# mlelarge/graph_neural_net

Hardware: AMD Instinct MI355X
Metric: graph-pairs/sec FGNN fwd+bwd, N=50 regular pairs (higher is better)
Workload: dtype f32

## Files before the change

### graph_neural_net_amd/_lib.py

```python
import ctypes as C
import os

import torch

_HERE = os.path.dirname(os.path.abspath(__file__))
LIB_PATH = os.environ.get('FGNN_LIB') or os.path.join(_HERE, 'libfgnn_hip.so')

FGNN_H = 32
FGNN_TILE = 32
FGNN_MAX_DEPTH = 3
FGNN_RANGE_WG = 256
FGNN_LSAP_MAX_N = 2048
FGNN_MAX_LEVELS = 64
FGNN_QAP_MAX_N = 256
FGNN_QAPW_MAX_N = 256
FGNN_SEED_MAX_N = 256
FGNN_SINKHORN_LDS_MAX_N = 192
FGNN_RESTART_STREAM = 9
FGNN_RESTART_MAX_R = 64
FGNN_RESTART_MAX_STARTS = 65535
FGNN_SPECTRAL_MAX_N = 256
FGNN_SPECTRAL_MAX_POWERS = 8
FGNN_PLANTED_MAX_N = 256
FGNN_SCORE_SPLIT = 4
# ... 54 lines not shown

class MlpBwdArgs(C.Structure):
    _fields_ = [('G', C.c_int), ('N', C.c_int), ('depth', C.c_int),
                ('nvalid', C.c_void_p),
                ('a', Slab), ('b', Slab),
                ('W', C.c_void_p * FGNN_MAX_DEPTH),
                ('bias', C.c_void_p * FGNN_MAX_DEPTH),
                ('dy', C.c_void_p), ('dgstride', C.c_longlong), ('ldd', C.c_longlong),
                ('z', C.c_void_p), ('zgstride', C.c_longlong), ('ldz', C.c_longlong),
                ('coef', C.c_void_p), ('s12', C.c_void_p), ('znrm', C.c_void_p),
                ('dxa', C.c_void_p), ('dxa_gstride', C.c_longlong), ('dxa_ld', C.c_longlong),
                ('dxb', C.c_void_p), ('dxb_gstride', C.c_longlong), ('dxb_ld', C.c_longlong),
                ('accumulate_a', C.c_int), ('accumulate_b', C.c_int),
                ('wpart', C.c_void_p), ('s12part', C.c_void_p), ('packed', C.c_void_p),
                ('s12tiles', C.c_void_p), ('s12_out', C.c_void_p), ('xbits', C.c_void_p), ('xdeg', C.c_void_p),
                ('ranges', C.c_void_p), ('cu_share', C.c_int)]


class Slab16(C.Structure):
    _fields_ = [('ptr', C.c_void_p), ('gstride', C.c_longlong), ('ldp', C.c_longlong), ('C', C.c_int),
                ('nrm', C.c_void_p), ('beta', C.c_void_p)]


class MlpFwd16Args(C.Structure):
    _fields_ = [('G', C.c_int), ('N', C.c_int), ('ldr', C.c_int), ('depth', C.c_int), ('nmlp', C.c_int),
                ('nvalid', C.c_void_p),
                ('a', Slab16), ('b', Slab16),
                ('z', C.c_void_p * 2), ('ldz', C.c_longlong),
                ('part', C.c_void_p * 2), ('cnt', C.c_void_p), ('packed', C.c_void_p), ('ranges', C.c_void_p)]


# ... 151 lines not shown
    'fgnn_block1_struct_supported': [_I, _I, _I],
    'fgnn_block1_struct_table_floats': [_I],
    'fgnn_block1_struct_ws_floats': [_I, _I],
    'fgnn_block1_struct_rows': [_I, _I],
    'fgnn_block1_struct_fwd': [_VP, _VP, _I, _I, _VP, _VP, _VP, _VP, _VP, C.c_float, _VP, _VP, _VP, _LL, _LL, _VP, _VP, _VP, _VP, _VP, _VP, _VP],
    'fgnn_block1_struct_bwd': [_VP, _VP, _I, _I, _VP, _VP, _VP, _VP, _VP, _VP, _VP, _VP, _LL, _LL, _VP, _VP, _VP, _VP, _VP, _VP],
    'fgnn_block1_struct_fwd_pack': [_VP, _VP, _I, _I, _VP, _VP, _VP, _VP, _VP, C.c_float, _VP, _VP, _VP, _LL, _LL, _VP, _VP, _VP, _VP, _VP, _VP, _VP, _I, _VP],
    'fgnn_block1_struct_fwd16_pack': [_VP, _VP, _I, _I, _I, _VP, _VP, _VP, _VP, _VP, C.c_float, _VP, _VP, _VP, _LL, _LL, _VP, _VP, _VP, _VP, _VP, _VP, _VP, _I, _VP],
    'fgnn_block1_struct_fwd16': [_VP, _VP, _I, _I, _I, _VP, _VP, _VP, _VP, _VP, C.c_float, _VP, _VP, _VP, _LL, _LL, _VP, _VP, _VP, _VP, _VP, _VP, _VP],
    'fgnn_block1_struct_bwd16': [_VP, _VP, _I, _I, _I, _VP, _VP, _VP, _VP, _VP, _VP, _VP, _VP, _LL, _LL, _VP, _VP, _VP, _VP, _VP, _VP],
    'fgnn_mlp_bwd_coef_tiles_supported': [_I, _I],
    'fgnn_mlp_param_count': [_I, _I],
    'fgnn_reduce_partials': [_VP, _I, _I, _VP, _VP],
    'fgnn_chan_matmul_bwd': [C.POINTER(Slab), C.POINTER(Slab), _VP, _LL, _LL, _VP, _I, _I, _VP, _VP, _LL, _LL, _VP, _VP, _VP],
    'fgnn_chan_matmul_bwd_ord': [C.POINTER(Slab), C.POINTER(Slab), _VP, _LL, _LL, _VP, _I, _I, _VP, _VP, _LL, _LL, _VP, _VP, _VP, _I, _VP],
    'fgnn_sum_scale': [_VP, _I, _I, _F, _VP, _VP],
    'fgnn_adam_step': [_VP, _VP, _VP, _VP, _I, C.c_double, C.c_double, C.c_double, C.c_double, _I, C.c_double, _VP],
    'fgnn_adam_step_dev': [_VP, _VP, _VP, _VP, _I, _VP, _VP, _VP],
    'fgnn_grad_guard': [_VP, _I, _VP, _VP, _VP],
    'fgnn_adam_step_guarded': [_VP, _VP, _VP, _VP, _I, _VP, _VP, _VP, _VP],
    'fgnn_expand_adjacency': [_VP, _VP, _I, _I, _VP, _VP],
    'fgnn_pack_adjacency': [_VP, _VP, _I, _I, _VP, _VP, _VP],
    'fgnn_pack_adjacency_ld': [_VP, _VP, _I, _I, _I, _VP, _VP, _VP],
    'fgnn_pack_adjacency_pair': [_VP, _VP, _VP, _VP, _I, _I, _I, _VP, _VP, _VP, _VP, _VP],
    'fgnn_adjacency_degree': [_VP, _VP, _I, _I, _VP, _VP],
    'fgnn_accuracy_max': [_VP, _VP, _I, _I, _VP, _VP],
    'fgnn_lsap_accuracy': [_VP, _LL, _I, _VP, _I, _I, _VP, _VP, _VP],
    'fgnn_pairgen_supported': [_I, _I, _I],
    'fgnn_pairgen': [C.POINTER(PairgenArgs), _VP],
    'fgnn_pairgen_indexed': [C.POINTER(PairgenArgs), _VP, _VP],
# ... 170 lines not shown
```

### graph_neural_net_amd/csrc/fgnn_bwd32.h

```cpp
#pragma once
#include "fgnn_common.h"

namespace {

constexpr int BWD_WG = 256;
constexpr int NW = 8;
constexpr int NP = 4;
static_assert(BWD_WG == FGNN_RANGE_WG, "fgnn_ragged_tile_ranges splits for the backward grid");

DEVI float4 coef_from_sums(const float4 n, const float2 sv, float nv) {
    const float m = nv * nv;
    float4 k;
    k.x = n.x;
    k.y = n.y;
    k.z = m > 0.f ? -n.y * sv.y * n.w / m : 0.f;
    k.w = m > 0.f ? -n.y * sv.x / m : 0.f;
    return k;
}
DEVI float4 coef_record(const fgnn_mlp_bwd_args &A, int g, int ch, int nv) {
    if (A.coef) return reinterpret_cast<const float4 *>(A.coef)[(long long)g * FGNN_H + ch];
    const float4 n = reinterpret_cast<const float4 *>(A.znrm)[(long long)g * FGNN_H + ch];
    const float2 sv = reinterpret_cast<const float2 *>(A.s12)[(long long)g * FGNN_H + ch];
    return coef_from_sums(n, sv, (float)nv);
}
// ... 35 lines not shown
        const int m = e >= PCOUNT / 4 ? 1 : 0, ee = e - m * (PCOUNT / 4);
        float4 a = part4[(4 * m) * (PCOUNT / 4) + ee];
#pragma unroll
        for (int w = 1; w < NP; ++w) {
            const float4 b = part4[(4 * m + w) * (PCOUNT / 4) + ee];
            a.x += b.x;
            a.y += b.y;
            a.z += b.z;
            a.w += b.w;
        }
        reinterpret_cast<float4 *>(P.m[m].wpart + (long long)blockIdx.x * PCOUNT)[ee] = a;
    }
}

inline int check_mlp_bwd_common(const fgnn_mlp_bwd_args *a, const char *fn, int tile_bits) {
    FGNN_CHECK(a->dy && a->z && a->wpart, "%s: missing dy/z/wpart", fn);
    FGNN_CHECK(a->coef || (a->s12 && a->znrm) || (a->s12tiles && a->znrm), "%s: need coef, or s12 + znrm, or s12tiles + znrm", fn);
    const long long lim = 0x7fffffffll / 4, G = a->G;
    FGNN_CHECK(G * a->a.gstride < lim && G * a->b.gstride < lim && G * a->dgstride < lim && G * a->zgstride < lim &&
               G * a->dxa_gstride < lim && G * a->dxb_gstride < lim,
               "%s: a tensor exceeds 2 GiB (32-bit buffer addressing); split the batch", fn);
    FGNN_CHECK(G * fgnn_tiles_per_graph(a->N) < (1ll << tile_bits), "%s: too many tiles", fn);
    FGNN_CHECK(BWD_WG == fgnn_mlp_bwd_num_workgroups(), "%s: workgroup count differs from fgnn_mlp_bwd", fn);
    return 0;
}
inline int check_pair_common(const fgnn_mlp_bwd_args *a1, const fgnn_mlp_bwd_args *a2, const char *fn, int tile_bits, bool dense_only) {
    FGNN_CHECK(a1 && a2, "%s: null args", fn);
    FGNN_CHECK(BWD_WG == fgnn_mlp_bwd_num_workgroups(), "%s: workgroup count differs from fgnn_mlp_bwd", fn);
    FGNN_CHECK(a1->G > 0 && a1->N > 0 && a1->G == a2->G && a1->N == a2->N && a1->depth == a2->depth,
               "%s: the two MLPs must share G, N and depth", fn);
    FGNN_CHECK((!dense_only || a1->a.ptr) && a1->a.ptr == a2->a.ptr && a1->a.C == a2->a.C && a1->a.gstride == a2->a.gstride &&
               a1->a.ldp == a2->a.ldp && a1->a.nrm == a2->a.nrm && a1->a.beta == a2->a.beta &&
               (dense_only || (a1->xbits == a2->xbits && a1->xdeg == a2->xdeg)) && a1->nvalid == a2->nvalid,
               "%s: the two MLPs must read the same input slab", fn);
    FGNN_CHECK(!a1->dxa && !a1->s12part, "%s: the input gradient and its tile sums belong to the SECOND argument block", fn);
    FGNN_CHECK(!a1->s12tiles && !a2->s12tiles, "%s: s12tiles is an mlp3 feature", fn);
    for (const fgnn_mlp_bwd_args *a : {a1, a2}) {
        FGNN_CHECK(a->dy && a->z && a->wpart, "%s: missing dy/z/wpart", fn);
        FGNN_CHECK(a->coef || (a->s12 && a->znrm), "%s: need coef, or s12 + znrm", fn);
        const long long lim = 0x7fffffffll / 4, G = a->G;
        FGNN_CHECK(G * a->a.gstride < lim && G * a->dgstride < lim && G * a->zgstride < lim && G * a->dxa_gstride < lim,
                   "%s: a tensor exceeds 2 GiB (32-bit buffer addressing); split the batch", fn);
    }
    FGNN_CHECK((long long)a1->G * fgnn_tiles_per_graph(a1->N) < (1ll << tile_bits), "%s: too many tiles", fn);
    return 0;
}

}
```

### graph_neural_net_amd/csrc/fgnn_bwd_t16.h

```cpp
#pragma once
#include "fgnn_t16.h"
#include "fgnn_pack.h"
#include "fgnn_bwd32.h"

namespace {

using namespace t16;

template <int CB, int IMAGES, int NSLOTS>
struct BwdT16Layout {
    static constexpr int DEPTH = 3;
    static constexpr PkBwd PK = pk_bwd(32, CB, DEPTH);
    static constexpr int OFF_W1 = PK.off_wh, OFF_WT1 = PK.off_wt, OFF_WT2 = PK.off_wt + 16;
    static constexpr int BIAS_F = PK.bias_f;
    static constexpr int WEIGHT_F = pk_pad_floats(PK.floats);
    static constexpr int NSLOT = NSLOTS;
    static constexpr int CIN = 32 + CB;
    static constexpr int PCOUNT = 32 * CIN + 32 + (DEPTH - 1) * (32 * 32 + 32);
    static constexpr int TILE_OFF = IMAGES * WEIGHT_F;
    static constexpr int TILE_END = TILE_OFF + NW * NSLOT * TILE_F;
    static constexpr int RED_F = NW * PCOUNT;
};


#define FGNN_T16_READ_RECORDS(norm)                                 \
    _Pragma("unroll") for (int s = 0; s < 8; ++s) {                 \
        const float4 k4 = rec[chan_s(s) + chan_q(q)];               \
        kx[s] = k4.x;                                               \
        ky[s] = k4.y;                                               \
        kz[s] = k4.z;                                               \
        kw[s] = k4.w;                                               \
        if (norm) {                                                 \
            const float4 n = rec[32 + chan_s(s) + chan_q(q)];       \
            mean[s] = n.x;                                          \
            av[s] = n.y;                                            \
        }                                                           \
    }

#define FGNN_T16_RECOMPUTE_HIDDEN(acc, h1, h2)                                              \
    _Pragma("unroll") for (int s = 0; s < 8; ++s) h1[s] = relu1(acc[s >> 2][s & 3]);        \
    stage8(S0, lane_base, h1);                                                              \
    load_bias(acc, wl + L::BIAS_F, 1, q);                                                   \
    gemm32<L::OFF_W1>(acc, wl, h1, lane);                                                   \
    _Pragma("unroll") for (int s = 0; s < 8; ++s) h2[s] = relu1(acc[s >> 2][s & 3]);        \
    stage8(S1, lane_base, h2);

#define FGNN_T16_DZ(dpre)                                                                                                   \
    _Pragma("unroll") for (int s = 0; s < 8; ++s) dpre[s] = fmaf(kz[s], zr[s] - kx[s], fmaf(ky[s], dyr[s], kw[s]));         \
    if (!full) {                                                                                                            \
        _Pragma("unroll") for (int s = 0; s < 8; ++s) dpre[s] = valid ? dpre[s] : 0.f;                                      \
    }

#define FGNN_T16_HIDDEN_BWD(OFF_WT, dpre, dW, db, Dt, In, h)                                                \
    {                                                                                                       \
        f32x4 a2[2];                                                                                        \
        a2[0] = a2[1] = zero4();                                                                            \
        gemm32<OFF_WT>(a2, wl, dpre, lane);                                                                 \
        wgrad16(dW, db, Dt, In, lane);                                                                      \
        _Pragma("unroll") for (int s = 0; s < 8; ++s) dpre[s] = h[s] > 0.f ? a2[s >> 2][s & 3] : 0.f;       \
    }

#define FGNN_T16_DB_BUTTERFLY(db0, db1, db2)            \
    _Pragma("unroll") for (int b = 0; b < 2; ++b) {     \
// ... 10 lines not shown
```

### graph_neural_net_amd/csrc/matmul.hip

```cpp
#include "fgnn_common.h"
#include "fgnn_norm.h"

namespace {

constexpr int TM = 64;
constexpr int LDS_LD = 65;

DEVI void stage_tile(float *lds, const float *mat, int N, int nv, int row0, int col0, const NormRec &nr, int tid) {
    if (row0 == 0 && col0 == 0 && N <= TM) {
        for (int e = tid; e < TM * TM; e += 256) lds[(e >> 6) * LDS_LD + (e & 63)] = 0.f;
        __syncthreads();
        const int P = N * N;
        for (int e = tid; e < P; e += 256) {
            const int r = e / N, c = e - r * N;
            float v = mat[e];
            const bool ok = r < nv && c < nv;
            v = ok ? (nr.on ? (v - nr.mean) * nr.a + nr.beta : v) : 0.f;
            lds[r * LDS_LD + c] = v;
        }
    } else {
        for (int e = tid; e < TM * TM; e += 256) {
            const int r = e >> 6, c = e & 63;
            const int gr = row0 + r, gc = col0 + c;
            float v = 0.f;
// ... 188 lines not shown
template <bool WANT_S>
DEVI void tile_to_global(const View &ov, int mat_off4, const float *lds, int N, const float (&u)[16], float &s1,
                         float &s2, int tid) {
    const int c = tid & 63, r0 = __builtin_amdgcn_readfirstlane(tid >> 6);
    const int voff = c < N ? (r0 * N + c) * 4 : OOB_OFF;
    const float *lp = lds + r0 * LDS_LD + c;
#pragma unroll
    for (int k = 0; k < 16; ++k) {
        const float t = lp[4 * k * LDS_LD];
        buf_store(t, ov, r0 + 4 * k < N ? voff : OOB_OFF, mat_off4 + k * 16 * N);
        if (WANT_S) {
            s1 += t;
            s2 += t * u[k];
        }
    }
}

DEVI void load_tile_raw(float (&x)[16], const View &v, int mat_off4, int N, int nv, int tid) {
    const int c = tid & 63, r0 = __builtin_amdgcn_readfirstlane(tid >> 6);
    const int voff = c < nv ? (r0 * N + c) * 4 : OOB_OFF;
#pragma unroll
    for (int k = 0; k < 16; ++k) {
        const int r = r0 + 4 * k;
        x[k] = buf_load(v, r < nv ? voff : OOB_OFF, mat_off4 + k * 16 * N);
    }
}
template <bool WANT_U>
DEVI void finish_tile(float (&v)[16], float (&u)[16], const float (&x)[16], int nv, const NormRec &nr, int tid) {
#pragma unroll
    for (int k = 0; k < 16; ++k) {
// ... 65 lines not shown
#pragma unroll
        for (int r = 0; r < 16; ++r) acc[r] = 0.f;
        if (32 * qi < N && 32 * qj < N) {
            const float *ap = As + (32 * qi + j) * LDS_LD + h;
            const float *bp = Bs + h * LDS_LD + 32 * qj + j;
            for (int k = 0; k < N; k += 2) acc = mfma32(ap[k], bp[k * LDS_LD], acc);
        }
        __syncthreads();
        frag_to_lds(As, 32 * qi, 32 * qj, acc, lane);
        __syncthreads();
        float s1 = 0.f, s2 = 0.f;
        tile_to_global<false>(vO, o_off, As, N, dummy, s1, s2, tid);
    }
}

__global__ __launch_bounds__(256, 4) void chan_matmul_bwd1_kernel(const fgnn_slab ya, const fgnn_slab yb,
                                                               const float *dm, long long dmg, long long ldm,
                                                               const int *nvalid, int N, int M, float *da, float *db,
                                                               long long ogstride, long long ldo, float *s12a,
                                                               float *s12b) {
    __shared__ float Bs[TM * LDS_LD];
    __shared__ float Ds[TM * LDS_LD];
    __shared__ float red[4][4];
    const int C = ya.C;
    const int tid = threadIdx.x, lane = tid & 63, wave = tid >> 6;
    const int qi = wave >> 1, qj = wave & 1;
    const int j = lane & 31, h = lane >> 5;
    NormRec none;
    none.on = false; none.mean = 0.f; none.a = 1.f; none.beta = 0.f;
    float xa[16], xb[16], xd[16], dummy[16];
// ... 33 lines not shown
            for (int k = 0; k < N; k += 2) accA = mfma32(ap[k], bp[k], accA);
        }
        __syncthreads();
        store_tile_lds(Bs, va, tid);
        __syncthreads();
        if (live) {
            const float *ap = Bs + h * LDS_LD + 32 * qi + j;
            const float *bp = Ds + h * LDS_LD + 32 * qj + j;
            for (int k = 0; k < N; k += 2) accB = mfma32(ap[k * LDS_LD], bp[k * LDS_LD], accB);
        }
        __syncthreads();
        frag_to_lds(Ds, 32 * qi, 32 * qj, accA, lane);
        frag_to_lds(Bs, 32 * qi, 32 * qj, accB, lane);
        __syncthreads();
        float sa1 = 0.f, sa2 = 0.f, sb1 = 0.f, sb2 = 0.f;
        if (s12a) {
            tile_to_global<true>(vOA, o_off, Ds, N, ua, sa1, sa2, tid);
            tile_to_global<true>(vOB, o_off, Bs, N, ub, sb1, sb2, tid);
            s12_epilogue(red, sa1, sa2, sb1, sb2, s12a, s12b, gc, tid);
        } else {
            tile_to_global<false>(vOA, o_off, Ds, N, dummy, sa1, sa2, tid);
            tile_to_global<false>(vOB, o_off, Bs, N, dummy, sb1, sb2, tid);
        }
    }
}


int g_mm_wave_variant = 1;
inline bool mm_wave_variant() { return (g_mm_wave_variant & 1) != 0; }
inline bool mm_narrow() { return (g_mm_wave_variant & 8) != 0; }
constexpr int WLD = 68;
// ... 654 lines not shown
extern "C" int fgnn_chan_matmul_bwd_ord(const fgnn_slab *ya, const fgnn_slab *yb, const float *dm, long long dmgstride,
                                        long long ldm, const int *nvalid, int G, int N, float *da, float *db,
                                        long long ogstride, long long ldo, float *s12a, float *s12b, const int *order,
                                        int fill, void *stream) {
    FGNN_CHECK(!order || nvalid, "fgnn_chan_matmul_bwd_ord: an order needs the nvalid it was derived from");
    FGNN_CHECK(ya && yb && dm && da && db && ya->ptr && yb->ptr, "fgnn_chan_matmul_bwd: null argument");
    FGNN_CHECK(ya->C == yb->C && ya->C > 0 && G > 0 && N > 0, "fgnn_chan_matmul_bwd: bad shapes");
    FGNN_CHECK((s12a == nullptr) == (s12b == nullptr), "fgnn_chan_matmul_bwd: s12a and s12b come together");
    FGNN_CHECK(!s12a || (ya->nrm && yb->nrm), "fgnn_chan_matmul_bwd: s12 outputs need normalised slabs");
    const int t = (N + TM - 1) / TM;
    const bool fused = s12a && t == 1;
    if (t == 1) {
        if (check_2gib("fgnn_chan_matmul_bwd", G, ya->gstride, yb->gstride, dmgstride)) return 1;
        FGNN_CHECK((long long)G * ogstride < 0x7fffffffll / 4, "fgnn_chan_matmul_bwd: output exceeds 2 GiB");
        const int M = G * ya->C;
        hipLaunchKernelGGL(chan_matmul_bwd1_kernel, dim3(M), dim3(256), 0, (hipStream_t)stream, *ya, *yb, dm,
                           dmgstride, ldm, nvalid, N, M, da, db, ogstride, ldo, s12a, s12b);
        FGNN_LAUNCH_CHECK();
        return 0;
    }
    if (big_path(N)) {
        if (check_2gib("fgnn_chan_matmul_bwd", G, ya->gstride, yb->gstride, dmgstride, ogstride)) return 1;
#define FGNN_BIG_BWD(MT)                                                                                              \
    {                                                                                                                 \
        static LdsAttrCache attr_cache;                                                                           \
        (void)fgnn_raise_lds(attr_cache, (const void *)chan_matmul_bwd_big_kernel<MT>, BigCfg<MT>::LDS_BYTES);                   \
        hipLaunchKernelGGL(chan_matmul_bwd_big_kernel<MT>, dim3(G * ya->C * (split ? 2 : 1)), dim3(BIG_THREADS),      \
                           BigCfg<MT>::LDS_BYTES, (hipStream_t)stream, *ya, *yb, dm, dmgstride, ldm, nvalid, N, G, da, \
                           db, ogstride, ldo, s12a, s12b, order, split, fill);                                            \
    }
        const int split = (order && (long long)G * ya->C <= BIG_SPLIT_MAX_MATRICES) ? 1 : 0;
// ... 2 lines not shown
#undef FGNN_BIG_BWD
        FGNN_LAUNCH_CHECK();
        return 0;
    }
    hipLaunchKernelGGL(chan_matmul_bwd_kernel, dim3(t, t, G * ya->C), dim3(256), 0, (hipStream_t)stream, *ya, *yb, dm,
                       dmgstride, ldm, nvalid, N, da, db, ogstride, ldo, fused ? s12a : nullptr, fused ? s12b : nullptr);
    FGNN_LAUNCH_CHECK();
    if (s12a && !fused) {
        int rc = fgnn_gn_bwd_stats(da, ogstride, ldo, ya->ptr, ya->gstride, ya->ldp, ya->nrm, nvalid, G, ya->C, N, s12a, stream);
        if (rc) return rc;
        rc = fgnn_gn_bwd_stats(db, ogstride, ldo, yb->ptr, yb->gstride, yb->ldp, yb->nrm, nvalid, G, yb->C, N, s12b, stream);
        if (rc) return rc;
    }
    return 0;
}
```

### graph_neural_net_amd/csrc/mlp_bwd_pair_t16.hip

```cpp
#include "fgnn_bwd_t16.h"

#ifdef FGNN_PHASES
__device__ unsigned long long *g_phase16_buf = nullptr;
#define PH_DECL unsigned long long ph_[16] = {0, 0, 0, 0, 0, 0, 0, 0, 0, 0, 0, 0, 0, 0, 0, 0}; unsigned long long ph_last_ = __builtin_amdgcn_s_memtime();
#define PH(k) { const unsigned long long t_ = __builtin_amdgcn_s_memtime(); ph_[k] += t_ - ph_last_; ph_last_ = t_; }
#define PH_FLUSH if (g_phase16_buf && (threadIdx.x & 63) == 0) { for (int k_ = 0; k_ < 16; ++k_) g_phase16_buf[((long long)blockIdx.x * NW + wv) * 16 + k_] = ph_[k_]; }
#else
#define PH_DECL
#define PH(k)
#define PH_FLUSH
#endif

namespace {

struct PairLayout16 : BwdT16Layout<0, 2, 4> {
    static constexpr int OFF_W0 = PK.off_w1a, OFF_WT0 = PK.off_wt0a;
    static constexpr int XCH_OFF = TILE_END;
    static constexpr int FLAG_OFF = XCH_OFF + NP * 1024;
    static constexpr int REC_OFF = FLAG_OFF + 4 * NP;
    static constexpr int LIVE_OFF = REC_OFF + NW * 256;
    static constexpr int MAIN_F = LIVE_OFF + LIVE_LIST_CAP + NW;
    static constexpr int LDS_F = MAIN_F > RED_F ? MAIN_F : RED_F;
};

template <bool SKIP, bool HAS_DX>
__global__ __launch_bounds__(64 * NW, 2) void mlp_bwd_pair_t16_kernel(const PairArgs P, const int tpg, const int total_tiles) {
    extern __shared__ __attribute__((aligned(16))) float smem[];
    using L = PairLayout16;
    const int lane = threadIdx.x & 63, wv = __builtin_amdgcn_readfirstlane(threadIdx.x >> 6);
    const int role = wv >> 2, pair = wv & 3;
    const int px = lane & 15, q = lane >> 4;
    const fgnn_mlp_bwd_args &A = P.m[role];
    const int P2 = A.N * A.N;
    const View va = make_view(A.a.ptr, A.a.gstride, A.a.ldp, A.G);
    const View vdy = make_view(A.dy, A.dgstride, A.ldd, A.G);
    const View vz = make_view(A.z, A.zgstride, A.ldz, A.G);
    const View vdx = make_view(P.m[1].dxa, P.m[1].dxa_gstride, P.m[1].dxa_ld, P.m[1].G);

    PH_DECL
    if (role == 1) __builtin_amdgcn_s_setprio(1);
// ... 23 lines not shown
    pk_glds<NW>(smem, P.m[0].packed, L::WEIGHT_F, wv, lane);
    pk_glds<NW>(smem + L::WEIGHT_F, P.m[1].packed, L::WEIGHT_F, wv, lane);
    PH(15)

    float mean[8], av[8], beta[8], kx[8], ky[8], kz[8], kw[8];
#pragma unroll
    for (int s = 0; s < 8; ++s) {
        mean[s] = 0.f;
        av[s] = 1.f;
        beta[s] = normA && A.a.beta ? A.a.beta[chan(s, 0) + chan_q(q)] : 0.f;
        kx[s] = ky[s] = kz[s] = kw[s] = 0.f;
    }
    float4 *rec = reinterpret_cast<float4 *>(smem + L::REC_OFF) + wv * 64;
    auto fetch_records = [&](int g, int nv) {
        if (lane < 32) {
            rec[lane] = coef_record(A, g, lane, nv);
            if (normA) rec[32 + lane] = reinterpret_cast<const float4 *>(A.a.nrm)[(long long)g * A.a.C + lane];
        }
    };
    auto read_records = [&]() { FGNN_T16_READ_RECORDS(normA) };

    float xa[8], dyr[8], zr[8], oldr[8];
#pragma unroll
    for (int s = 0; s < 8; ++s) oldr[s] = 0.f;
    int cached_g = -1, cur_nv = A.N;
    int tile = T0 + pair;
    int live_cnt = 0;
    if constexpr (SKIP) tile = __builtin_amdgcn_readfirstlane(next_owned_live_tile_p(T0, T1, live_cnt, pair, NP, tpg, FGNN_TILE, A.N, A.nvalid));
    int hf = 0;
    {
        const bool act = tile < T1;
        const int g = __builtin_amdgcn_readfirstlane(act ? tile / tpg : 0);
        const int p = (act ? tile - g * tpg : 0) * 32 + px;
        const bool inb0 = act && p < P2;
        load8(xa, va, lane_voff(va, q, p, inb0), g * va.gs4);
// ... 5 lines not shown
    }
    PH(12)
    if (threadIdx.x < 4 * NP) reinterpret_cast<int *>(smem + L::FLAG_OFF)[threadIdx.x] = 0;
    PH(13)
    int *live_list = reinterpret_cast<int *>(smem + L::LIVE_OFF);
    int nlive = 0, li = pair;
    if constexpr (SKIP) nlive = build_live_list(live_list, live_list + LIVE_LIST_CAP, T0, T1, tpg, FGNN_TILE, A.N, A.nvalid, threadIdx.x, 64 * NW);
    const bool use_list = SKIP && nlive <= LIVE_LIST_CAP;
    __syncthreads();
    {
        const bool act = tile < T1;
        const int g = __builtin_amdgcn_readfirstlane(act ? tile / tpg : 0);
        const int p = (act ? tile - g * tpg : 0) * 32 + px;
        const bool inb0 = act && p < P2;
        load8(dyr, vdy, lane_voff(vdy, q, p, inb0), g * vdy.gs4);
        load8(zr, vz, lane_voff(vz, q, p, inb0), g * vz.gs4);
        if (has_dx) load8(oldr, vdx, lane_voff(vdx, q, p, inb0 && rmw && role == 0), g * vdx.gs4);
    }
    if (cached_g >= 0) read_records();
    PH(9)

    int hk = 0;
    float es1[8], es2[8];
#pragma unroll
    for (int s = 0; s < 8; ++s) es1[s] = es2[s] = 0.f;
    while (tile < T1) {
        int tnext = tile + NP;
        if constexpr (SKIP) {
            if (hf == 1) {
                if (use_list) {
                    li += NP;
// ... 39 lines not shown
            {
                float ya[8];
#pragma unroll
                for (int s = 0; s < 8; ++s) {
                    u[s] = xa[s] - mean[s];
                    ya[s] = u[s] * av[s] + beta[s];
                }
                stage8(XA, lane_base, ya);
                f32x4 acc[2];
                load_bias(acc, wl + L::BIAS_F, 0, q);
                gemm32<L::OFF_W0>(acc, wl, ya, lane);
                FGNN_T16_RECOMPUTE_HIDDEN(acc, h1, h2)
            }
            PH(1)
            float dpre[8];
            FGNN_T16_DZ(dpre)
            stage8(S2, lane_base, dpre);
            load8(dyr, vdy, lane_voff(vdy, q, np, ninb), ng * vdy.gs4);
            load8(zr, vz, lane_voff(vz, q, np, ninb), ng * vz.gs4);
            PH(2)
            __builtin_amdgcn_sched_barrier(0);
            FGNN_T16_HIDDEN_BWD(L::OFF_WT2, dpre, dW2, db2, S2, S1, h2)
            PH(3)
            __builtin_amdgcn_sched_barrier(0);
            stage8(S1, lane_base, dpre);
            FGNN_T16_HIDDEN_BWD(L::OFF_WT1, dpre, dW1, db1, S1, S0, h1)
            PH(4)
            __builtin_amdgcn_sched_barrier(0);
            stage8(S2, lane_base, dpre);
            __builtin_amdgcn_sched_barrier(0);
#pragma unroll
            for (int s = 0; s < 8; ++s) dx[s >> 2][s & 3] = oldr[s];
            load8(xa, va, lane_voff(va, q, np, ninb), ng * va.gs4);
            if (has_dx) load8(oldr, vdx, lane_voff(vdx, q, np, ninb && rmw && role == 0), ng * vdx.gs4);
// ... 92 lines not shown
            if (q == 0) {
                red[off + 1024 + row_chan(px)] = db[0];
                red[off + 1024 + row_chan(16 + px)] = db[1];
            }
        };
        put(0, dW0, db0);
        put(1056, dW1, db1);
        put(2112, dW2, db2);
    }
    __syncthreads();
    sum_pair_partials<PCOUNT>(smem, P);
    PH(11)
    PH_FLUSH
}

template <bool SKIP, bool HAS_DX>
int launch_pair16(const fgnn_mlp_bwd_args *a1, const fgnn_mlp_bwd_args *a2, int tpg, int total, hipStream_t st) {
    constexpr int LDS = PairLayout16::LDS_F * 4;
    static_assert(LDS <= 160 * 1024, "LDS budget");
    static LdsAttrCache attr_cache;
    (void)fgnn_raise_lds(attr_cache, (const void *)mlp_bwd_pair_t16_kernel<SKIP, HAS_DX>, LDS);
    PairArgs P;
    P.m[0] = *a1;
    P.m[1] = *a2;
    hipLaunchKernelGGL((mlp_bwd_pair_t16_kernel<SKIP, HAS_DX>), dim3(a1->cu_share == 2 && !SKIP ? BWD_WG / 2 : BWD_WG), dim3(64 * NW), LDS, st, P, tpg,
                       total);
    FGNN_LAUNCH_CHECK();
    return 0;
}

}

#ifdef FGNN_PHASES
extern "C" int fgnn_debug_phase_buffer_t16(void *p) { return hipMemcpyToSymbol(HIP_SYMBOL(g_phase16_buf), &p, sizeof(p)) == hipSuccess ? 0 : 1; }
#endif

extern "C" int fgnn_mlp_bwd_pair_t16(const fgnn_mlp_bwd_args *a1, const fgnn_mlp_bwd_args *a2, void *stream) {
    if (check_pair_common(a1, a2, "fgnn_mlp_bwd_pair_t16", 29, true)) return 1;
    FGNN_CHECK(a1->depth == 3 && a1->a.C == 32 && a1->b.C == 0 && a2->b.C == 0 && !a1->xbits && !a2->xbits,
               "fgnn_mlp_bwd_pair_t16: built for depth 3 and ONE dense input slab of 32 channels (got depth %d, %d + %d); use fgnn_mlp_bwd_pair",
               a1->depth, a1->a.C, a1->b.C);
    FGNN_CHECK(a1->ranges == a2->ranges && (!a1->ranges || a1->nvalid), "fgnn_mlp_bwd_pair_t16: both MLPs take the same ranges (with nvalid)");
    FGNN_CHECK(a1->packed && a2->packed, "fgnn_mlp_bwd_pair_t16: needs both operand images (fgnn_pack_operands, kind 5)");
    FGNN_CHECK(a1->N <= 256, "fgnn_mlp_bwd_pair_t16: N <= 256 (division-free pixel decode)");
    const int tpg = fgnn_tiles_per_graph(a1->N);
    const long long total = (long long)a1->G * tpg;
    hipStream_t st = (hipStream_t)stream;
    if (a2->dxa) return a1->ranges ? launch_pair16<true, true>(a1, a2, tpg, (int)total, st) : launch_pair16<false, true>(a1, a2, tpg, (int)total, st);
    return a1->ranges ? launch_pair16<true, false>(a1, a2, tpg, (int)total, st) : launch_pair16<false, false>(a1, a2, tpg, (int)total, st);
}
```

### graph_neural_net_amd/engine.py

```python
import ctypes as C
import os

import torch

from . import _lib
from .engine_base import EngineBase

EPS = 1e-05


class ParamLayout:

    def __init__(self, original_features_num=2, num_blocks=4, in_features=32, out_features=32, depth_of_mlp=3):
        if in_features != _lib.FGNN_H or out_features != _lib.FGNN_H:
            raise RuntimeError('the fused engine is built for in_features = out_features = 32 (got %d, %d); other widths '
                               'run through the per-layer modules (layers.MlpBlock_Real)' % (in_features, out_features))
        if not 1 <= depth_of_mlp <= _lib.FGNN_MAX_DEPTH:
            raise RuntimeError('depth_of_mlp must be in 1..%d' % _lib.FGNN_MAX_DEPTH)
        if original_features_num not in (2, 32):
            raise RuntimeError('the fused engine is built for original_features_num = 2 or 32 (got %d); other widths run '
                               'through the per-layer modules (layers.MlpBlock_Real)' % original_features_num)
        self.c0 = original_features_num
        self.num_blocks = num_blocks
        self.depth = depth_of_mlp
# ... 100 lines not shown
        return len(self._items)

    def __iter__(self):
        return iter(list(self._items))

    def values(self):
        return [e for e, _ in self._items.values()]


class FgnnEngine(EngineBase):
    SKIP_PADDING_TILES = True
    MM_ORDER = True
    PAIR_BWD = os.environ.get('FGNN_PAIR_BWD', '1') != '0'
    PACK_IN_STRUCT = os.environ.get('FGNN_PACK_IN_STRUCT', '1') != '0'
    T16 = os.environ.get('FGNN_T16', 'pair,bwd')

    MFMA = os.environ.get('FGNN_MFMA', 'f32')

    BLOCK1 = os.environ.get('FGNN_BLOCK1', 'generic')
    GN_FINALIZE = ('fgnn_gn_finalize', 'fgnn_gn_finalize2')

    def __init__(self, layout, G, N, device, ragged=False, cu_share=0, mfma=None, block1=None):
        _lib.load()
        self.T16 = type(self).T16
        self.cu_share = int(cu_share)
        mfma = self.MFMA if mfma is None else mfma
        if mfma not in ('f32', 'x3'):
            raise ValueError("mfma must be 'f32' or 'x3' (got %r)" % (mfma,))
        self.x3 = (mfma == 'x3' and not ragged and layout.depth == 3 and layout.c0 in (2, 32))
        block1 = self.BLOCK1 if block1 is None else block1
# ... 218 lines not shown
        W = self._bwd
        _lib.call('fgnn_gn_bwd_coef', _lib.ptr(W['s12'][kj]), _lib.ptr(self.nrm[kj]), self._nv(), self.G, 32, self.N,
                  _lib.ptr(W['coef'][slot]), None, None, _lib.stream_ptr())

    def _mlp_bwd(self, params, k, j, a, b, dy, coef, dxa, dxb, acc_a, acc_b, emit=False, dx_strides=None):
        args = self._mlp_bwd_args(params, k, j, a, b, dy, coef, dxa, dxb, acc_a, acc_b, emit, dx_strides)
        entry = 'fgnn_mlp_bwd_x3' if (self.x3 and j != 3) else 'fgnn_mlp_bwd'
        if j == 3 and b is not None and self._t16_bwd3(b.C) and _lib.load().fgnn_mlp_bwd_t16_supported(C.byref(args)):
            entry = 'fgnn_mlp_bwd_t16'
        elif self._packs[('b', k, j)][0] == 5:
            args.packed = None
        _lib.call(entry, C.byref(args), _lib.stream_ptr(),
                  tag='mlp_bwd[cin=%d,dx=%d]' % (a.C + (b.C if b is not None else 0),
                                                (a.C if dxa is not None else 0) + (b.C if (b is not None and dxb is not None) else 0)))

    def _mlp_bwd_pair(self, params, k, sin, din, emit):
        W = self._bwd
        a1 = self._mlp_bwd_args(params, k, 1, sin, None, W['dy1'], None, None, None, False, False, False, None)
        a2 = self._mlp_bwd_args(params, k, 2, sin, None, W['dy2'], None, din, None, True, False, emit, None)
        entry = 'fgnn_mlp_bwd_pair_x3' if self.x3 else ('fgnn_mlp_bwd_pair_t16' if self._t16_pair(sin.C) else 'fgnn_mlp_bwd_pair')
        _lib.call(entry, C.byref(a1), C.byref(a2), _lib.stream_ptr(),
                  tag='mlp_bwd_pair[cin=%d,dx=%d]' % (sin.C, sin.C if din is not None else 0))

    def _mlp_bwd_args(self, params, k, j, a, b, dy, coef, dxa, dxb, acc_a, acc_b, emit, dx_strides):
        L = self.layout
        W = self._bwd
        rec = L.mlp[(k, j)]
        gs = 32 * self.ldp
        args = _lib.MlpBwdArgs()
        args.G, args.N, args.depth = self.G, self.N, L.depth
        args.nvalid = self.nvalid.data_ptr() if self.nvalid is not None else None
        args.a = a
        if b is not None:
            args.b = b
# ... 45 lines not shown
            din = None if first else W['dy'][(K - k + 1) % 2]
            dxs = None
            if first and dx is not None:
                if self.xbits is not None or self.x3 or tuple(dx.shape) != (self.G, L.c0, self.N, self.N) or dx.dtype != torch.float32 \
                        or not dx.is_contiguous():
                    raise RuntimeError('FgnnEngine: the input gradient needs a dense fp32 input, the fp32-MFMA kernels (mfma="f32") '
                                       'and a contiguous (G, c0, N, N) fp32 dx')
                din, dxs = dx, (L.c0 * self.P, self.P)
            self._mlp_bwd(params, k, 3, self._slab_raw(self.mult[k]), sin, dy,
                          None if k == K else ('tiles' if in_prologue else W['coef'][2]), W['dmult'], din, False, False, dx_strides=dxs)
            if first and self.struct1 and self.xbits is not None and dxs is None:
                self._struct_bwd(params)
                dy = din
                continue
            ya, yb = self._slab_z(k, 1, params), self._slab_z(k, 2, params)
            _lib.call('fgnn_chan_matmul_bwd_ord', C.byref(ya), C.byref(yb), _lib.ptr(W['dmult']), gs, self.ldp,
                      self._nv(), self.G, self.N, _lib.ptr(W['dy1']), _lib.ptr(W['dy2']), gs, self.ldp,
                      _lib.ptr(W['s12'][(k, 1)]), _lib.ptr(W['s12'][(k, 2)]),
                      _lib.ptr(self.mm_order) if self.mm_order is not None else None, self._fill(), st, tag='fgnn_chan_matmul_bwd')
            if first:
                W['struct_rows'] = 0
            if self.PAIR_BWD and dxs is None and L.depth == 3 and sin.C in (2, 32):
                self._mlp_bwd_pair(params, k, sin, din, emit=not first)
            else:
                self._mlp_bwd(params, k, 1, sin, None, W['dy1'], None, din, None, True, False, dx_strides=dxs)
                self._mlp_bwd(params, k, 2, sin, None, W['dy2'], None, din, None, True, False, emit=not first, dx_strides=dxs)
            if not first and not in_prologue:
                _lib.call('fgnn_gn_bwd_coef_tiles', _lib.ptr(W['s12part']), _lib.ptr(self.nrm[(k - 1, 3)]), self._nv(),
                          self.G, 32, self.N, _lib.ptr(W['s12'][(k - 1, 3)]), _lib.ptr(W['coef'][2]), st)
            dy = din
        if finalize:
            self.grad_finalize(grads)
        return grads

    def relu_decisions(self, params=None):
        L, G, N, P = self.layout, self.G, self.N, self.P
        out = {}
        bit = torch.arange(32, device=self.device, dtype=torch.int32)
# ... 38 lines not shown
```

### include/fgnn_hip.h

```cpp
#ifndef FGNN_HIP_H
#define FGNN_HIP_H

#ifdef __cplusplus
extern "C" {
#endif

#define FGNN_H 32
#define FGNN_TILE 32
#define FGNN_MAX_DEPTH 3

typedef struct {
    const float *ptr;
    long long gstride;
    long long ldp;
    int C;
    const float *nrm;
    const float *beta;
} fgnn_slab;

const char *fgnn_last_error(void);
int fgnn_version(void);
int fgnn_tiles_per_graph(int N);
int fgnn_mlp_bwd_num_workgroups(void);

// ... 201 lines not shown
    const float *coef;
    const float *s12;
    const float *znrm;
    float *dxa; long long dxa_gstride, dxa_ld;
    float *dxb; long long dxb_gstride, dxb_ld;
    int accumulate_a, accumulate_b;
    float *wpart;
    float *s12part;
    const float *packed;
    const float *s12tiles;
    float *s12_out;
    const unsigned *xbits;
    const float *xdeg;
    const int *ranges;
    int cu_share;
} fgnn_mlp_bwd_args;
int fgnn_mlp_bwd(const fgnn_mlp_bwd_args *args, void *stream);
int fgnn_mlp_bwd_x3(const fgnn_mlp_bwd_args *args, void *stream);
int fgnn_mlp_bwd_pair(const fgnn_mlp_bwd_args *m1, const fgnn_mlp_bwd_args *m2, void *stream);
int fgnn_mlp_bwd_pair_x3(const fgnn_mlp_bwd_args *m1, const fgnn_mlp_bwd_args *m2, void *stream);
int fgnn_mlp_bwd_t16_supported(const fgnn_mlp_bwd_args *args);
int fgnn_mlp_bwd_t16(const fgnn_mlp_bwd_args *args, void *stream);
int fgnn_mlp_bwd_pair_t16(const fgnn_mlp_bwd_args *m1, const fgnn_mlp_bwd_args *m2, void *stream);
#define FGNN_BWD_COEF_GRAPHS 4
int fgnn_mlp_bwd_coef_tiles_supported(int G, int N);
int fgnn_mlp_param_count(int Cin, int depth);
int fgnn_reduce_partials(const float *wpart, int num_wg, int count, float *out, void *stream);

#define FGNN_MAX_GRAD_JOBS 16
typedef struct {
// ... 2 lines not shown
    int rows;
    float scale;
    const float *scale_dev;
} fgnn_grad_job;
int fgnn_grad_finalize(const fgnn_grad_job *jobs, int njobs, int num_wg, int G, int C, void *stream);
int fgnn_inv_node_count(const int *nvalid, int B, float *out, void *stream);

int fgnn_chan_matmul_bwd(const fgnn_slab *ya, const fgnn_slab *yb, const float *dm, long long dmgstride, long long ldm,
                         const int *nvalid, int G, int N,
                         float *da, float *db, long long ogstride, long long ldo,
                         float *s12a ,
                         float *s12b , void *stream);
int fgnn_chan_matmul_bwd_ord(const fgnn_slab *ya, const fgnn_slab *yb, const float *dm, long long dmgstride, long long ldm,
                             const int *nvalid, int G, int N, float *da, float *db, long long ogstride, long long ldo,
                             float *s12a, float *s12b, const int *order, int fill , void *stream);

int fgnn_adam_step(float *params, const float *grads, float *exp_avg, float *exp_avg_sq, int n, double lr,
                   double beta1, double beta2, double eps, int step, double grad_scale, void *stream);
int fgnn_adam_step_dev(float *params, const float *grads, float *exp_avg, float *exp_avg_sq, int n,
                       const double *hp, int *state, void *stream);
#define FGNN_GUARD_MAX_PARTS 64
#define FGNN_GUARD_SKIP_NONFINITE 1
#define FGNN_GUARD_NONFINITE 1
typedef struct {
    double max_norm;
    double norm;
    double coef;
    int flags;
    int skipped;
    int arrivals;
// ... 364 lines not shown
```

Baseline: 42240.

## Hand the normalisation backward from channel-matmul epilogue to the pair MLP backward

The channel-matmul backward kernel gains a template variant that reduces the per-channel tile sums in its epilogue, derives the normalisation-backward coefficients in place, and writes the pre-norm gradient dz directly. The t16 pair MLP backward gets a matching DZIN variant that reads this gradient as-is, skipping the z loads and coefficient records. This removes one global read of z and the coef arithmetic from the MLP backward. The path is limited to constant-size batches with N no larger than one tile, and it adds a new struct field and validation checks.

```diff
diff --git a/graph_neural_net_amd/_lib.py b/graph_neural_net_amd/_lib.py
--- a/graph_neural_net_amd/_lib.py
+++ b/graph_neural_net_amd/_lib.py
@@ -92,7 +92,7 @@
                 ('accumulate_a', C.c_int), ('accumulate_b', C.c_int),
                 ('wpart', C.c_void_p), ('s12part', C.c_void_p), ('packed', C.c_void_p),
                 ('s12tiles', C.c_void_p), ('s12_out', C.c_void_p), ('xbits', C.c_void_p), ('xdeg', C.c_void_p),
-                ('ranges', C.c_void_p), ('cu_share', C.c_int)]
+                ('ranges', C.c_void_p), ('cu_share', C.c_int), ('dy_is_dz', C.c_int)]
 
 
 class Slab16(C.Structure):
@@ -274,6 +274,8 @@
     'fgnn_reduce_partials': [_VP, _I, _I, _VP, _VP],
     'fgnn_chan_matmul_bwd': [C.POINTER(Slab), C.POINTER(Slab), _VP, _LL, _LL, _VP, _I, _I, _VP, _VP, _LL, _LL, _VP, _VP, _VP],
     'fgnn_chan_matmul_bwd_ord': [C.POINTER(Slab), C.POINTER(Slab), _VP, _LL, _LL, _VP, _I, _I, _VP, _VP, _LL, _LL, _VP, _VP, _VP, _I, _VP],
+    'fgnn_chan_matmul_bwd_dz_supported': [_I],
+    'fgnn_chan_matmul_bwd_dz_ord': [C.POINTER(Slab), C.POINTER(Slab), _VP, _LL, _LL, _VP, _I, _I, _VP, _VP, _LL, _LL, _VP, _VP, _VP, _I, _VP],
     'fgnn_sum_scale': [_VP, _I, _I, _F, _VP, _VP],
     'fgnn_adam_step': [_VP, _VP, _VP, _VP, _I, C.c_double, C.c_double, C.c_double, C.c_double, _I, C.c_double, _VP],
     'fgnn_adam_step_dev': [_VP, _VP, _VP, _VP, _I, _VP, _VP, _VP],
diff --git a/graph_neural_net_amd/csrc/fgnn_bwd32.h b/graph_neural_net_amd/csrc/fgnn_bwd32.h
--- a/graph_neural_net_amd/csrc/fgnn_bwd32.h
+++ b/graph_neural_net_amd/csrc/fgnn_bwd32.h
@@ -73,6 +73,7 @@
 }
 
 inline int check_mlp_bwd_common(const fgnn_mlp_bwd_args *a, const char *fn, int tile_bits) {
+    FGNN_CHECK(!a->dy_is_dz, "%s: dy_is_dz is built in fgnn_mlp_bwd_pair_t16 only", fn);
     FGNN_CHECK(a->dy && a->z && a->wpart, "%s: missing dy/z/wpart", fn);
     FGNN_CHECK(a->coef || (a->s12 && a->znrm) || (a->s12tiles && a->znrm), "%s: need coef, or s12 + znrm, or s12tiles + znrm", fn);
     const long long lim = 0x7fffffffll / 4, G = a->G;
@@ -83,8 +84,11 @@
     FGNN_CHECK(BWD_WG == fgnn_mlp_bwd_num_workgroups(), "%s: workgroup count differs from fgnn_mlp_bwd", fn);
     return 0;
 }
-inline int check_pair_common(const fgnn_mlp_bwd_args *a1, const fgnn_mlp_bwd_args *a2, const char *fn, int tile_bits, bool dense_only) {
+inline int check_pair_common(const fgnn_mlp_bwd_args *a1, const fgnn_mlp_bwd_args *a2, const char *fn, int tile_bits, bool dense_only,
+                             bool dz_ok = false) {
     FGNN_CHECK(a1 && a2, "%s: null args", fn);
+    FGNN_CHECK(dz_ok || (!a1->dy_is_dz && !a2->dy_is_dz), "%s: dy_is_dz is built in fgnn_mlp_bwd_pair_t16 only", fn);
+    FGNN_CHECK(!a1->dy_is_dz == !a2->dy_is_dz, "%s: dy_is_dz is set in both argument blocks or in neither", fn);
     FGNN_CHECK(BWD_WG == fgnn_mlp_bwd_num_workgroups(), "%s: workgroup count differs from fgnn_mlp_bwd", fn);
     FGNN_CHECK(a1->G > 0 && a1->N > 0 && a1->G == a2->G && a1->N == a2->N && a1->depth == a2->depth,
                "%s: the two MLPs must share G, N and depth", fn);
@@ -95,8 +99,8 @@
     FGNN_CHECK(!a1->dxa && !a1->s12part, "%s: the input gradient and its tile sums belong to the SECOND argument block", fn);
     FGNN_CHECK(!a1->s12tiles && !a2->s12tiles, "%s: s12tiles is an mlp3 feature", fn);
     for (const fgnn_mlp_bwd_args *a : {a1, a2}) {
-        FGNN_CHECK(a->dy && a->z && a->wpart, "%s: missing dy/z/wpart", fn);
-        FGNN_CHECK(a->coef || (a->s12 && a->znrm), "%s: need coef, or s12 + znrm", fn);
+        FGNN_CHECK(a->dy && (a->z || a->dy_is_dz) && a->wpart, "%s: missing dy/z/wpart", fn);
+        FGNN_CHECK(a->dy_is_dz || a->coef || (a->s12 && a->znrm), "%s: need coef, or s12 + znrm", fn);
         const long long lim = 0x7fffffffll / 4, G = a->G;
         FGNN_CHECK(G * a->a.gstride < lim && G * a->dgstride < lim && G * a->zgstride < lim && G * a->dxa_gstride < lim,
                    "%s: a tensor exceeds 2 GiB (32-bit buffer addressing); split the batch", fn);
diff --git a/graph_neural_net_amd/csrc/fgnn_bwd_t16.h b/graph_neural_net_amd/csrc/fgnn_bwd_t16.h
--- a/graph_neural_net_amd/csrc/fgnn_bwd_t16.h
+++ b/graph_neural_net_amd/csrc/fgnn_bwd_t16.h
@@ -37,6 +37,15 @@
         }                                                           \
     }
 
+#define FGNN_T16_READ_NRM(norm)                                     \
+    if (norm) {                                                     \
+        _Pragma("unroll") for (int s = 0; s < 8; ++s) {             \
+            const float4 n = rec[32 + chan_s(s) + chan_q(q)];       \
+            mean[s] = n.x;                                          \
+            av[s] = n.y;                                            \
+        }                                                           \
+    }
+
 #define FGNN_T16_RECOMPUTE_HIDDEN(acc, h1, h2)                                              \
     _Pragma("unroll") for (int s = 0; s < 8; ++s) h1[s] = relu1(acc[s >> 2][s & 3]);        \
     stage8(S0, lane_base, h1);                                                              \
@@ -47,6 +56,12 @@
 
 #define FGNN_T16_DZ(dpre)                                                                                                   \
     _Pragma("unroll") for (int s = 0; s < 8; ++s) dpre[s] = fmaf(kz[s], zr[s] - kx[s], fmaf(ky[s], dyr[s], kw[s]));         \
+    if (!full) {                                                                                                            \
+        _Pragma("unroll") for (int s = 0; s < 8; ++s) dpre[s] = valid ? dpre[s] : 0.f;                                      \
+    }
+
+#define FGNN_T16_DZ_GIVEN(dpre)                                                                                             \
+    _Pragma("unroll") for (int s = 0; s < 8; ++s) dpre[s] = dyr[s];                                                         \
     if (!full) {                                                                                                            \
         _Pragma("unroll") for (int s = 0; s < 8; ++s) dpre[s] = valid ? dpre[s] : 0.f;                                      \
     }
diff --git a/graph_neural_net_amd/csrc/matmul.hip b/graph_neural_net_amd/csrc/matmul.hip
--- a/graph_neural_net_amd/csrc/matmul.hip
+++ b/graph_neural_net_amd/csrc/matmul.hip
@@ -1,5 +1,6 @@
 #include "fgnn_common.h"
 #include "fgnn_norm.h"
+#include "fgnn_bwd32.h"
 
 namespace {
 
@@ -226,6 +227,24 @@
             s2 += t * u[k];
         }
     }
+}
+
+DEVI void tile_sums(float (&t)[16], const float *lds, const float (&u)[16], float &s1, float &s2, int tid) {
+    const int c = tid & 63, r0 = __builtin_amdgcn_readfirstlane(tid >> 6);
+    const float *lp = lds + r0 * LDS_LD + c;
+#pragma unroll
+    for (int k = 0; k < 16; ++k) {
+        t[k] = lp[4 * k * LDS_LD];
+        s1 += t[k];
+        s2 += t[k] * u[k];
+    }
+}
+DEVI void dz_to_global(const View &ov, int mat_off4, int N, const float (&t)[16], const float (&u)[16], const float4 k4, int tid) {
+    const int c = tid & 63, r0 = __builtin_amdgcn_readfirstlane(tid >> 6);
+    const int voff = c < N ? (r0 * N + c) * 4 : OOB_OFF;
+#pragma unroll
+    for (int k = 0; k < 16; ++k)
+        buf_store(fmaf(k4.z, u[k], fmaf(k4.y, t[k], k4.w)), ov, r0 + 4 * k < N ? voff : OOB_OFF, mat_off4 + k * 16 * N);
 }
 
 DEVI void load_tile_raw(float (&x)[16], const View &v, int mat_off4, int N, int nv, int tid) {
@@ -321,6 +340,7 @@
     }
 }
 
+template <bool DZ>
 __global__ __launch_bounds__(256, 4) void chan_matmul_bwd1_kernel(const fgnn_slab ya, const fgnn_slab yb,
                                                                const float *dm, long long dmg, long long ldm,
                                                                const int *nvalid, int N, int M, float *da, float *db,
@@ -384,7 +404,21 @@
         frag_to_lds(Bs, 32 * qi, 32 * qj, accB, lane);
         __syncthreads();
         float sa1 = 0.f, sa2 = 0.f, sb1 = 0.f, sb2 = 0.f;
-        if (s12a) {
+        if constexpr (DZ) {
+            float ta[16], tb[16];
+            tile_sums(ta, Ds, ua, sa1, sa2, tid);
+            tile_sums(tb, Bs, ub, sb1, sb2, tid);
+            s12_epilogue(red, sa1, sa2, sb1, sb2, s12a, s12b, gc, tid);
+            const float nvf = (float)nv;
+            const float4 ka = coef_from_sums(reinterpret_cast<const float4 *>(ya.nrm)[(long long)g * C + c],
+                                             make_float2((red[0][0] + red[1][0]) + (red[2][0] + red[3][0]),
+                                                         (red[0][1] + red[1][1]) + (red[2][1] + red[3][1])), nvf);
+            const float4 kb = coef_from_sums(reinterpret_cast<const float4 *>(yb.nrm)[(long long)g * C + c],
+                                             make_float2((red[0][2] + red[1][2]) + (red[2][2] + red[3][2]),
+                                                         (red[0][3] + red[1][3]) + (red[2][3] + red[3][3])), nvf);
+            dz_to_global(vOA, o_off, N, ta, ua, ka, tid);
+            dz_to_global(vOB, o_off, N, tb, ub, kb, tid);
+        } else if (s12a) {
             tile_to_global<true>(vOA, o_off, Ds, N, ua, sa1, sa2, tid);
             tile_to_global<true>(vOB, o_off, Bs, N, ub, sb1, sb2, tid);
             s12_epilogue(red, sa1, sa2, sb1, sb2, s12a, s12b, gc, tid);
@@ -1069,7 +1103,7 @@
         if (check_2gib("fgnn_chan_matmul_bwd", G, ya->gstride, yb->gstride, dmgstride)) return 1;
         FGNN_CHECK((long long)G * ogstride < 0x7fffffffll / 4, "fgnn_chan_matmul_bwd: output exceeds 2 GiB");
         const int M = G * ya->C;
-        hipLaunchKernelGGL(chan_matmul_bwd1_kernel, dim3(M), dim3(256), 0, (hipStream_t)stream, *ya, *yb, dm,
+        hipLaunchKernelGGL(chan_matmul_bwd1_kernel<false>, dim3(M), dim3(256), 0, (hipStream_t)stream, *ya, *yb, dm,
                            dmgstride, ldm, nvalid, N, M, da, db, ogstride, ldo, s12a, s12b);
         FGNN_LAUNCH_CHECK();
         return 0;
@@ -1102,3 +1136,24 @@
     }
     return 0;
 }
+
+extern "C" int fgnn_chan_matmul_bwd_dz_supported(int N) { return (N > 0 && N <= TM) ? 1 : 0; }
+
+extern "C" int fgnn_chan_matmul_bwd_dz_ord(const fgnn_slab *ya, const fgnn_slab *yb, const float *dm, long long dmgstride,
+                                           long long ldm, const int *nvalid, int G, int N, float *dza, float *dzb,
+                                           long long ogstride, long long ldo, float *s12a, float *s12b, const int *order,
+                                           int fill, void *stream) {
+    (void)fill;
+    FGNN_CHECK(ya && yb && dm && dza && dzb && ya->ptr && yb->ptr, "fgnn_chan_matmul_bwd_dz: null argument");
+    FGNN_CHECK(ya->C == yb->C && ya->C > 0 && G > 0 && N > 0, "fgnn_chan_matmul_bwd_dz: bad shapes");
+    FGNN_CHECK(fgnn_chan_matmul_bwd_dz_supported(N), "fgnn_chan_matmul_bwd_dz: N=%d > %d (use fgnn_chan_matmul_bwd_ord)", N, TM);
+    FGNN_CHECK(s12a && s12b && ya->nrm && yb->nrm, "fgnn_chan_matmul_bwd_dz: dz needs the s12 outputs and normalised slabs");
+    FGNN_CHECK(!nvalid && !order, "fgnn_chan_matmul_bwd_dz: built for constant-size batches (no nvalid, no order)");
+    if (check_2gib("fgnn_chan_matmul_bwd_dz", G, ya->gstride, yb->gstride, dmgstride)) return 1;
+    FGNN_CHECK((long long)G * ogstride < 0x7fffffffll / 4, "fgnn_chan_matmul_bwd_dz: output exceeds 2 GiB");
+    const int M = G * ya->C;
+    hipLaunchKernelGGL(chan_matmul_bwd1_kernel<true>, dim3(M), dim3(256), 0, (hipStream_t)stream, *ya, *yb, dm, dmgstride, ldm,
+                       nvalid, N, M, dza, dzb, ogstride, ldo, s12a, s12b);
+    FGNN_LAUNCH_CHECK();
+    return 0;
+}
diff --git a/graph_neural_net_amd/csrc/mlp_bwd_pair_t16.hip b/graph_neural_net_amd/csrc/mlp_bwd_pair_t16.hip
--- a/graph_neural_net_amd/csrc/mlp_bwd_pair_t16.hip
+++ b/graph_neural_net_amd/csrc/mlp_bwd_pair_t16.hip
@@ -23,7 +23,7 @@
     static constexpr int LDS_F = MAIN_F > RED_F ? MAIN_F : RED_F;
 };
 
-template <bool SKIP, bool HAS_DX>
+template <bool SKIP, bool HAS_DX, bool DZIN>
 __global__ __launch_bounds__(64 * NW, 2) void mlp_bwd_pair_t16_kernel(const PairArgs P, const int tpg, const int total_tiles) {
     extern __shared__ __attribute__((aligned(16))) float smem[];
     using L = PairLayout16;
@@ -77,11 +77,17 @@
     float4 *rec = reinterpret_cast<float4 *>(smem + L::REC_OFF) + wv * 64;
     auto fetch_records = [&](int g, int nv) {
         if (lane < 32) {
-            rec[lane] = coef_record(A, g, lane, nv);
+            if constexpr (!DZIN) rec[lane] = coef_record(A, g, lane, nv);
             if (normA) rec[32 + lane] = reinterpret_cast<const float4 *>(A.a.nrm)[(long long)g * A.a.C + lane];
         }
     };
-    auto read_records = [&]() { FGNN_T16_READ_RECORDS(normA) };
+    auto read_records = [&]() {
+        if constexpr (DZIN) {
+            FGNN_T16_READ_NRM(normA)
+        } else {
+            FGNN_T16_READ_RECORDS(normA)
+        }
+    };
 
     float xa[8], dyr[8], zr[8], oldr[8];
 #pragma unroll
@@ -117,7 +123,7 @@
         const int p = (act ? tile - g * tpg : 0) * 32 + px;
         const bool inb0 = act && p < P2;
         load8(dyr, vdy, lane_voff(vdy, q, p, inb0), g * vdy.gs4);
-        load8(zr, vz, lane_voff(vz, q, p, inb0), g * vz.gs4);
+        if constexpr (!DZIN) load8(zr, vz, lane_voff(vz, q, p, inb0), g * vz.gs4);
         if (has_dx) load8(oldr, vdx, lane_voff(vdx, q, p, inb0 && rmw && role == 0), g * vdx.gs4);
     }
     if (cached_g >= 0) read_records();
@@ -187,10 +193,14 @@
             }
             PH(1)
             float dpre[8];
-            FGNN_T16_DZ(dpre)
+            if constexpr (DZIN) {
+                FGNN_T16_DZ_GIVEN(dpre)
+            } else {
+                FGNN_T16_DZ(dpre)
+            }
             stage8(S2, lane_base, dpre);
             load8(dyr, vdy, lane_voff(vdy, q, np, ninb), ng * vdy.gs4);
-            load8(zr, vz, lane_voff(vz, q, np, ninb), ng * vz.gs4);
+            if constexpr (!DZIN) load8(zr, vz, lane_voff(vz, q, np, ninb), ng * vz.gs4);
             PH(2)
             __builtin_amdgcn_sched_barrier(0);
             FGNN_T16_HIDDEN_BWD(L::OFF_WT2, dpre, dW2, db2, S2, S1, h2)
@@ -313,16 +323,16 @@
     PH_FLUSH
 }
 
-template <bool SKIP, bool HAS_DX>
+template <bool SKIP, bool HAS_DX, bool DZIN = false>
 int launch_pair16(const fgnn_mlp_bwd_args *a1, const fgnn_mlp_bwd_args *a2, int tpg, int total, hipStream_t st) {
     constexpr int LDS = PairLayout16::LDS_F * 4;
     static_assert(LDS <= 160 * 1024, "LDS budget");
     static LdsAttrCache attr_cache;
-    (void)fgnn_raise_lds(attr_cache, (const void *)mlp_bwd_pair_t16_kernel<SKIP, HAS_DX>, LDS);
+    (void)fgnn_raise_lds(attr_cache, (const void *)mlp_bwd_pair_t16_kernel<SKIP, HAS_DX, DZIN>, LDS);
     PairArgs P;
     P.m[0] = *a1;
     P.m[1] = *a2;
-    hipLaunchKernelGGL((mlp_bwd_pair_t16_kernel<SKIP, HAS_DX>), dim3(a1->cu_share == 2 && !SKIP ? BWD_WG / 2 : BWD_WG), dim3(64 * NW), LDS, st, P, tpg,
+    hipLaunchKernelGGL((mlp_bwd_pair_t16_kernel<SKIP, HAS_DX, DZIN>), dim3(a1->cu_share == 2 && !SKIP ? BWD_WG / 2 : BWD_WG), dim3(64 * NW), LDS, st, P, tpg,
                        total);
     FGNN_LAUNCH_CHECK();
     return 0;
@@ -335,7 +345,7 @@
 #endif
 
 extern "C" int fgnn_mlp_bwd_pair_t16(const fgnn_mlp_bwd_args *a1, const fgnn_mlp_bwd_args *a2, void *stream) {
-    if (check_pair_common(a1, a2, "fgnn_mlp_bwd_pair_t16", 29, true)) return 1;
+    if (check_pair_common(a1, a2, "fgnn_mlp_bwd_pair_t16", 29, true, true)) return 1;
     FGNN_CHECK(a1->depth == 3 && a1->a.C == 32 && a1->b.C == 0 && a2->b.C == 0 && !a1->xbits && !a2->xbits,
                "fgnn_mlp_bwd_pair_t16: built for depth 3 and ONE dense input slab of 32 channels (got depth %d, %d + %d); use fgnn_mlp_bwd_pair",
                a1->depth, a1->a.C, a1->b.C);
@@ -345,6 +355,10 @@
     const int tpg = fgnn_tiles_per_graph(a1->N);
     const long long total = (long long)a1->G * tpg;
     hipStream_t st = (hipStream_t)stream;
+    if (a1->dy_is_dz) {
+        FGNN_CHECK(!a1->nvalid && !a1->ranges, "fgnn_mlp_bwd_pair_t16: dy_is_dz is built for constant-size batches (no nvalid, no ranges)");
+        return a2->dxa ? launch_pair16<false, true, true>(a1, a2, tpg, (int)total, st) : launch_pair16<false, false, true>(a1, a2, tpg, (int)total, st);
+    }
     if (a2->dxa) return a1->ranges ? launch_pair16<true, true>(a1, a2, tpg, (int)total, st) : launch_pair16<false, true>(a1, a2, tpg, (int)total, st);
     return a1->ranges ? launch_pair16<true, false>(a1, a2, tpg, (int)total, st) : launch_pair16<false, false>(a1, a2, tpg, (int)total, st);
 }
diff --git a/graph_neural_net_amd/engine.py b/graph_neural_net_amd/engine.py
--- a/graph_neural_net_amd/engine.py
+++ b/graph_neural_net_amd/engine.py
@@ -138,6 +138,7 @@
     PAIR_BWD = os.environ.get('FGNN_PAIR_BWD', '1') != '0'
     PACK_IN_STRUCT = os.environ.get('FGNN_PACK_IN_STRUCT', '1') != '0'
     T16 = os.environ.get('FGNN_T16', 'pair,bwd')
+    DZ_HANDOVER = os.environ.get('FGNN_DZ_HANDOVER', '1') != '0'
 
     MFMA = os.environ.get('FGNN_MFMA', 'f32')
 
@@ -386,10 +387,15 @@
                   tag='mlp_bwd[cin=%d,dx=%d]' % (a.C + (b.C if b is not None else 0),
                                                 (a.C if dxa is not None else 0) + (b.C if (b is not None and dxb is not None) else 0)))
 
-    def _mlp_bwd_pair(self, params, k, sin, din, emit):
+    def _dz_handover(self, sin, dxs):
+        return (self.DZ_HANDOVER and self.PAIR_BWD and dxs is None and self.layout.depth == 3 and self._t16_pair(sin.C)
+                and self.nvalid is None and bool(_lib.load().fgnn_chan_matmul_bwd_dz_supported(self.N)))
+
+    def _mlp_bwd_pair(self, params, k, sin, din, emit, dz=False):
         W = self._bwd
         a1 = self._mlp_bwd_args(params, k, 1, sin, None, W['dy1'], None, None, None, False, False, False, None)
         a2 = self._mlp_bwd_args(params, k, 2, sin, None, W['dy2'], None, din, None, True, False, emit, None)
+        a1.dy_is_dz = a2.dy_is_dz = int(dz)
         entry = 'fgnn_mlp_bwd_pair_x3' if self.x3 else ('fgnn_mlp_bwd_pair_t16' if self._t16_pair(sin.C) else 'fgnn_mlp_bwd_pair')
         _lib.call(entry, C.byref(a1), C.byref(a2), _lib.stream_ptr(),
                   tag='mlp_bwd_pair[cin=%d,dx=%d]' % (sin.C, sin.C if din is not None else 0))
@@ -465,14 +471,16 @@
                 dy = din
                 continue
             ya, yb = self._slab_z(k, 1, params), self._slab_z(k, 2, params)
-            _lib.call('fgnn_chan_matmul_bwd_ord', C.byref(ya), C.byref(yb), _lib.ptr(W['dmult']), gs, self.ldp,
+            dz = self._dz_handover(sin, dxs)
+            _lib.call('fgnn_chan_matmul_bwd_dz_ord' if dz else 'fgnn_chan_matmul_bwd_ord',
+                      C.byref(ya), C.byref(yb), _lib.ptr(W['dmult']), gs, self.ldp,
                       self._nv(), self.G, self.N, _lib.ptr(W['dy1']), _lib.ptr(W['dy2']), gs, self.ldp,
                       _lib.ptr(W['s12'][(k, 1)]), _lib.ptr(W['s12'][(k, 2)]),
                       _lib.ptr(self.mm_order) if self.mm_order is not None else None, self._fill(), st, tag='fgnn_chan_matmul_bwd')
             if first:
                 W['struct_rows'] = 0
             if self.PAIR_BWD and dxs is None and L.depth == 3 and sin.C in (2, 32):
-                self._mlp_bwd_pair(params, k, sin, din, emit=not first)
+                self._mlp_bwd_pair(params, k, sin, din, emit=not first, dz=dz)
             else:
                 self._mlp_bwd(params, k, 1, sin, None, W['dy1'], None, din, None, True, False, dx_strides=dxs)
                 self._mlp_bwd(params, k, 2, sin, None, W['dy2'], None, din, None, True, False, emit=not first, dx_strides=dxs)
diff --git a/include/fgnn_hip.h b/include/fgnn_hip.h
--- a/include/fgnn_hip.h
+++ b/include/fgnn_hip.h
@@ -239,6 +239,7 @@
     const float *xdeg;
     const int *ranges;
     int cu_share;
+    int dy_is_dz;
 } fgnn_mlp_bwd_args;
 int fgnn_mlp_bwd(const fgnn_mlp_bwd_args *args, void *stream);
 int fgnn_mlp_bwd_x3(const fgnn_mlp_bwd_args *args, void *stream);
@@ -271,6 +272,10 @@
 int fgnn_chan_matmul_bwd_ord(const fgnn_slab *ya, const fgnn_slab *yb, const float *dm, long long dmgstride, long long ldm,
                              const int *nvalid, int G, int N, float *da, float *db, long long ogstride, long long ldo,
                              float *s12a, float *s12b, const int *order, int fill , void *stream);
+int fgnn_chan_matmul_bwd_dz_supported(int N);
+int fgnn_chan_matmul_bwd_dz_ord(const fgnn_slab *ya, const fgnn_slab *yb, const float *dm, long long dmgstride, long long ldm,
+                                const int *nvalid, int G, int N, float *dza, float *dzb, long long ogstride, long long ldo,
+                                float *s12a, float *s12b, const int *order, int fill, void *stream);
 
 int fgnn_adam_step(float *params, const float *grads, float *exp_avg, float *exp_avg_sq, int n, double lr,
                    double beta1, double beta2, double eps, int step, double grad_scale, void *stream);
```

Result: no change. 42190 (median of 2 runs) (-0.1%).
